# yoxu515/aot-benchmark

Hardware: NVIDIA H100
Metric: frames/sec (480p, 10 obj) (higher is better)
Workload: dtype f32

## Files before the change

### aot_benchmark_b200/csrc/conv_tc.cu

```cuda
#include <type_traits>

#include "common.cuh"
#include "tc_common.cuh"

namespace aotb {
namespace tc {

constexpr int CONV_A_BYTES = 128 * 128;

template <int BN>
__device__ __forceinline__ void wgmma_conv(float* acc, uint64_t a, uint64_t b) {
    if (BN == 256) wgmma_ss_n256(acc, a, b, 1u);
    else if (BN == 128) wgmma_ss_n128(acc, a, b, 1u);
    else wgmma_ss_n64(acc, a, b, 1u);
}

template <int BN>
__device__ __forceinline__ void conv_acc_to_staging(const float* acc, float* stg, int ld) {
    const int warp = threadIdx.x >> 5, lane = threadIdx.x & 31;
    const int row0 = (warp >> 2) * 64 + (warp & 3) * 16 + (lane >> 2), cq = (lane & 3) * 2;
#pragma unroll
    for (int j = 0; j < BN / 2; j += 2)
        *reinterpret_cast<float2*>(stg + (row0 + 8 * ((j >> 1) & 1)) * ld + 8 * (j >> 2) + cq) = make_float2(acc[j], acc[j + 1]);
}

struct ConvTcArgs {
    const float* in;
    const float* bias;
    const float* wscale;
    const float* res;
    float* out;
    int B, H, W, Cin, ldin;
    int Ho, Wo, Cout, ldout, ldres;
    int KH, KW, stride, pad;
    int M, mtiles, nchunks;
    int act;
    int splits;
    int spin;
    int const_w;
    long long* prof;
};

constexpr int AOTB_CONV_CONST_WEIGHTS = 256;
static int g_conv_tiling = 0;
static int g_conv_grid_cap = 0;

struct RowInfo { int pix_base, iy0, ix0, valid; };

template <int BN, int S, int NB>
__device__ __forceinline__ void conv_finish_tile(const ConvTcArgs& a, const uint8_t* smem, int tid, int m0, int n0, int zrank) {
    constexpr int LD = BN + 4, C4 = BN / 4, RSTEP = 256 / C4, ROWS = 128 / S, ITERS = ROWS / RSTEP;
    constexpr int B = NB < ITERS ? NB : ITERS;
    static_assert(ITERS >= 1 && ITERS % B == 0, "finish tiling");
    const int c = (tid % C4) * 4, n = n0 + c;
    const int r0 = zrank * ROWS + tid / C4;
    const float4 b4 = a.bias ? __ldg(reinterpret_cast<const float4*>(a.bias + n)) : make_float4(0.f, 0.f, 0.f, 0.f);
    const float4 s4 = a.wscale ? __ldg(reinterpret_cast<const float4*>(a.wscale + n)) : make_float4(1.f, 1.f, 1.f, 1.f);
    const float* lbase = reinterpret_cast<const float*>(smem) + r0 * LD + c;
    const uint32_t sbase = smem_u32(lbase);
#pragma unroll 1
    for (int i0 = 0; i0 < ITERS; i0 += B) {
        float4 v[B][S], rs[B];
#pragma unroll
        for (int b = 0; b < B; ++b) {
            const int ro = (i0 + b) * RSTEP;
            if (S == 1) {
                v[b][0] = *reinterpret_cast<const float4*>(lbase + ro * LD);
            } else {
#pragma unroll
                for (int z = 0; z < S; ++z) v[b][z] = dsmem_ld_f4(dsmem_addr(sbase + (uint32_t)(ro * LD) * 4u, (uint32_t)z));
            }
            const int m = m0 + r0 + ro;
            rs[b] = (a.res && m < a.M) ? *reinterpret_cast<const float4*>(a.res + (size_t)m * a.ldres + n)
                                       : make_float4(0.f, 0.f, 0.f, 0.f);
        }
#pragma unroll
        for (int b = 0; b < B; ++b) {
            float4 o = v[b][0];
#pragma unroll
            for (int z = 1; z < S; ++z) { o.x += v[b][z].x; o.y += v[b][z].y; o.z += v[b][z].z; o.w += v[b][z].w; }
            o.x = fmaf(o.x, s4.x, b4.x); o.y = fmaf(o.y, s4.y, b4.y); o.z = fmaf(o.z, s4.z, b4.z); o.w = fmaf(o.w, s4.w, b4.w);
            o.x += rs[b].x; o.y += rs[b].y; o.z += rs[b].z; o.w += rs[b].w;
            o.x = apply_act(o.x, a.act); o.y = apply_act(o.y, a.act);
            o.z = apply_act(o.z, a.act); o.w = apply_act(o.w, a.act);
            const int m = m0 + r0 + (i0 + b) * RSTEP;
            if (m < a.M) *reinterpret_cast<float4*>(a.out + (size_t)m * a.ldout + n) = o;
        }
    }
}

__device__ __forceinline__ void prefetch_l1(const void* p) { asm volatile("prefetch.global.L1 [%0];" ::"l"(p)); }

template <int BN, int ACT>
__device__ __forceinline__ void conv_finish_frag(const ConvTcArgs& a, float* acc, const float* bs, int m0, int n0) {
    constexpr bool ROLL = ACT == ACT_GELU || ACT == ACT_SILU;
    constexpr int G = (ROLL || BN == 256) ? 1 : 8, NG = BN / 8, PF = 8;
    const int warp = threadIdx.x >> 5, lane = threadIdx.x & 31;
    const int r = m0 + (warp >> 2) * 64 + (warp & 3) * 16 + (lane >> 2);
    const int c = (lane & 3) * 2;
    const bool ok[2] = {r < a.M, r + 8 < a.M};
    auto res_at = [&](int h, int k) { return a.res + (size_t)(r + 8 * h) * a.ldres + n0 + c + 8 * k; };
    auto prefetch = [&](int k) {
        if (G == 1 && a.res && k < NG) {
            if (ok[0]) prefetch_l1(res_at(0, k));
            if (ok[1]) prefetch_l1(res_at(1, k));
        }
    };
    auto group = [&](int k, int h, float a0, float a1, float2 rs) {
        const int n = c + 8 * k;
        const float2 b2 = *reinterpret_cast<const float2*>(bs + n), s2 = *reinterpret_cast<const float2*>(bs + BN + n);
        float ox = fmaf(a0, s2.x, b2.x), oy = fmaf(a1, s2.y, b2.y);
        ox += rs.x; oy += rs.y;
        ox = apply_act(ox, ACT); oy = apply_act(oy, ACT);
        if (ok[h]) *reinterpret_cast<float2*>(a.out + (size_t)(r + 8 * h) * a.ldout + n0 + n) = make_float2(ox, oy);
    };
#pragma unroll
    for (int k = 0; k < PF; ++k) prefetch(k);
    if constexpr (ROLL) {
#pragma unroll 1
        for (int k = 0; k < NG; ++k) {
            prefetch(k + PF);
            float2 rs[2];
#pragma unroll
            for (int h = 0; h < 2; ++h)
                rs[h] = (a.res && ok[h]) ? *reinterpret_cast<const float2*>(res_at(h, k)) : make_float2(0.f, 0.f);
#pragma unroll
            for (int h = 0; h < 2; ++h) group(k, h, acc[2 * h], acc[2 * h + 1], rs[h]);
#pragma unroll
            for (int i = 0; i < BN / 2 - 4; ++i) acc[i] = acc[i + 4];
        }
    } else {
#pragma unroll
        for (int k0 = 0; k0 < NG; k0 += G) {
            prefetch(k0 + PF);
            float2 rs[G][2];
#pragma unroll
            for (int k = 0; k < G; ++k)
#pragma unroll
                for (int h = 0; h < 2; ++h)
                    rs[k][h] = (a.res && ok[h]) ? *reinterpret_cast<const float2*>(res_at(h, k0 + k)) : make_float2(0.f, 0.f);
#pragma unroll
            for (int k = 0; k < G; ++k)
#pragma unroll
                for (int h = 0; h < 2; ++h) group(k0 + k, h, acc[4 * (k0 + k) + 2 * h], acc[4 * (k0 + k) + 2 * h + 1], rs[k][h]);
        }
    }
}

template <int BN, int STAGES, bool SPLIT, bool PERSIST>
struct ConvSmem {
    static constexpr int A_BYTES = CONV_A_BYTES;
    static constexpr int B_BYTES = BN * 128;
    static constexpr int PARTS = SPLIT ? 2 : 1;
    static constexpr int STAGE_BYTES = PARTS * A_BYTES + PARTS * B_BYTES;
    static constexpr int STG_LD = BN + 4;
    static_assert(128 * STG_LD * 4 <= STAGES * STAGE_BYTES, "staging tile must fit in the operand stages");
    static constexpr int RTABLES = PERSIST ? 2 : 1, BS_FLOATS = PERSIST ? 2 * 2 * BN : 0;
    static constexpr int TOTAL = STAGES * STAGE_BYTES + RTABLES * 128 * (int)sizeof(RowInfo) + BS_FLOATS * 4 + 3 * STAGES * 8 + 1024;
    static_assert(TOTAL <= 227 * 1024, "shared memory of one CTA");
};

template <int BN, int STAGES, bool SPLIT, bool PERSIST>
__global__ void __launch_bounds__(384, 1)
conv_tc_kernel(const __grid_constant__ CUtensorMap tmWh, const __grid_constant__ CUtensorMap tmWl, const ConvTcArgs a) {
    using SM = ConvSmem<BN, STAGES, SPLIT, PERSIST>;
    extern __shared__ uint8_t smem_raw[];
    uint8_t* smem = reinterpret_cast<uint8_t*>((reinterpret_cast<uintptr_t>(smem_raw) + 1023) & ~(uintptr_t)1023);
    RowInfo* rinfo = reinterpret_cast<RowInfo*>(smem + STAGES * SM::STAGE_BYTES);
    float* bsm = reinterpret_cast<float*>(rinfo + SM::RTABLES * 128);
    uint64_t* a_full = reinterpret_cast<uint64_t*>(bsm + SM::BS_FLOATS);
    uint64_t* b_full = a_full + STAGES;
    uint64_t* s_free = b_full + STAGES;

    const int tid = threadIdx.x, warp = tid >> 5;
    const int ntn = a.Cout / BN, ntiles = a.mtiles * ntn;
    const int ntc = !PERSIST ? 1 : (int)blockIdx.x < ntiles ? (ntiles - 1 - (int)blockIdx.x) / (int)gridDim.x + 1 : 0;
    auto tile_m0 = [&](int j) {
        if constexpr (PERSIST) return ((int)(blockIdx.x + j * gridDim.x) / ntn) * 128;
// ... 70 lines not shown
                bs[tid] = a.bias ? __ldg(a.bias + n) : 0.f;
                bs[BN + tid] = a.wscale ? __ldg(a.wscale + n) : 1.f;
            }
#pragma unroll 1
            for (int it = 0; it < nloc; ++it, ++g) {
                const int s = g % STAGES;
                const uint32_t ph = (g / STAGES) & 1;
                mbar_wait_cp(&a_full[s], ph, a.spin);
                mbar_wait_cp(&b_full[s], ph, a.spin);
                if (g == 0 && tid == 0) stamp(3);
                const uint64_t so = (uint64_t)((s * SM::STAGE_BYTES) >> 4);
                const uint64_t ah = dA0 + so, al = ah + (SM::A_BYTES >> 4), bh = dB0 + so, bl = bh + (uint64_t)(SM::B_BYTES >> 4);
                reg_fence<BN / 2>(acc);
                wgmma_fence();
#pragma unroll
                for (int ks = 0; ks < 4; ++ks) {
                    wgmma_conv<BN>(acc, ah + 2 * ks, bh + 2 * ks);
                    if constexpr (SPLIT) {
                        wgmma_conv<BN>(acc, al + 2 * ks, bh + 2 * ks);
                        wgmma_conv<BN>(acc, ah + 2 * ks, bl + 2 * ks);
                    }
                }
                wgmma_commit();
                reg_fence<BN / 2>(acc);
                wgmma_wait<1>();
                if (it > 0) mbar_arrive_warp(&s_free[(g - 1) % STAGES]);
            }
            wgmma_wait<0>();
            reg_fence<BN / 2>(acc);
            if (tid == 0) { if (PERSIST && j == 0) stamp(10); stamp(4); }
            if constexpr (PERSIST) {
                if (nloc > 0) mbar_arrive_warp(&s_free[(g - 1) % STAGES]);
                asm volatile("bar.sync 1, 256;" ::: "memory");
                const int m0 = tile_m0(j), n0 = tile_n0(j);
                switch (a.act) {
                    case ACT_RELU: conv_finish_frag<BN, ACT_RELU>(a, acc, bs, m0, n0); break;
                    case ACT_GELU: conv_finish_frag<BN, ACT_GELU>(a, acc, bs, m0, n0); break;
                    case ACT_SILU: conv_finish_frag<BN, ACT_SILU>(a, acc, bs, m0, n0); break;
                    case ACT_RELU6: conv_finish_frag<BN, ACT_RELU6>(a, acc, bs, m0, n0); break;
                    default: conv_finish_frag<BN, ACT_NONE>(a, acc, bs, m0, n0); break;
                }
                if (tid == 0) { if (j == 0) stamp(8); stamp(9); }
            } else {
                asm volatile("bar.sync 1, 256;" ::: "memory");
                conv_acc_to_staging<BN>(acc, reinterpret_cast<float*>(smem), SM::STG_LD);
                if (tid == 0) stamp(6);
            }
        }
    } else {
        const int p = tid - 256, q = p & 15, rsub = p >> 4;
        const uint32_t soff = rsub * 128 + (((q >> 1) ^ rsub) << 4) + ((q & 1) << 3);
        const float4* in4 = reinterpret_cast<const float4*>(a.in);
        uint32_t off[16];
        int cur_tap = -1, c4 = 0;
        const RowInfo* rows = rinfo;
        auto load_half = [&](int h, auto part_c, float4* v) {
            constexpr int part = decltype(part_c)::value;
            if (part == 0) {
                const int g = h >> 1, j = PERSIST ? g / nloc : 0, it = g - j * nloc;
                if (PERSIST && it == 0) {
                    cur_tap = -1;
                    rows = rinfo + (j & 1) * 128;
                    if (j > 0) {
                        asm volatile("bar.sync 2, 128;" ::: "memory");
                        if (j + 1 < ntc) write_rows(j + 1, p);
                    }
                }
                const int kc = kbeg + it;
                int tap, c0;
                if (cpt > 0) { tap = kc / cpt; c0 = ((kc - tap * cpt) << 6) + q * 4; }
                else { const int k = kc * 64 + q * 4; tap = k / a.Cin; c0 = k - tap * a.Cin; }
                c4 = c0 >> 2;
                if (tap != cur_tap) {
                    cur_tap = tap;
// ... 63 lines not shown
                if (h + 4 < nh) load_half(h + 4, P0{}, v1);
                store_half(h + 2, P0{}, v2);
                if (h + 5 < nh) load_half(h + 5, P1{}, v2);
                store_half(h + 3, P1{}, v0);
            }
            if (h + 4 < nh) {
                if (h + 6 < nh) load_half(h + 6, P0{}, v0);
                store_half(h + 4, P0{}, v1);
                if (h + 7 < nh) load_half(h + 7, P1{}, v1);
                store_half(h + 5, P1{}, v2);
            }
        }
        if (p == 0) stamp(5);
    }
    if constexpr (!PERSIST) {
        __syncwarp();
        cluster_sync_all();
        if (tid == 0) stamp(8);
        if (warp < 8) {
            const int zr = (int)blockIdx.z, m0 = tile_m0(0), n0 = tile_n0(0);
            if (a.splits == 2) conv_finish_tile<BN, 2, 4>(a, smem, tid, m0, n0, zr);
            else if (a.splits == 4) conv_finish_tile<BN, 4, 2>(a, smem, tid, m0, n0, zr);
            else conv_finish_tile<BN, 8, 2>(a, smem, tid, m0, n0, zr);
        }
        if (tid == 0) stamp(9);
        __syncwarp();
        cluster_sync_all();
    } else if (tid == 0 && prof) {
        prof[11] = ntc;
    }
    if (tid == 0) stamp(7);
}

static int make_tmap_weights(CUtensorMap* out, const void* base, int Kpad, int Cout, int BN) {
    PFN_encodeTiled fn = tensor_map_encoder();
    if (!fn) return AOTB_ERR_CUDA;
    cuuint64_t dims[2] = {(cuuint64_t)Kpad, (cuuint64_t)Cout};
    cuuint64_t strides[1] = {(cuuint64_t)Kpad * 2};
    cuuint32_t box[2] = {64, (cuuint32_t)BN};
    cuuint32_t estr[2] = {1, 1};
    CUresult r = fn(out, CU_TENSOR_MAP_DATA_TYPE_FLOAT16, 2, const_cast<void*>(base), dims, strides, box, estr,
                    CU_TENSOR_MAP_INTERLEAVE_NONE, CU_TENSOR_MAP_SWIZZLE_128B, CU_TENSOR_MAP_L2_PROMOTION_L2_256B,
                    CU_TENSOR_MAP_FLOAT_OOB_FILL_NONE);
    if (r != CUDA_SUCCESS) {
        set_error("cuTensorMapEncodeTiled(weights) failed (%d)", (int)r);
        return AOTB_ERR_CUDA;
    }
    return AOTB_OK;
}

static int sm_count() {
    static int n = 0;
    if (n == 0) {
        int dev = 0;
        if (cudaGetDevice(&dev) != cudaSuccess || cudaDeviceGetAttribute(&n, cudaDevAttrMultiProcessorCount, dev) != cudaSuccess)
            n = 132;
    }
    return n;
}

static dim3 conv_grid(const ConvTcArgs& a, int BN) {
    if (a.splits > 1) return dim3(a.mtiles, a.Cout / BN, a.splits);
    const int cap = g_conv_grid_cap > 0 ? g_conv_grid_cap : sm_count();
    return dim3(min(a.mtiles * (a.Cout / BN), cap), 1, 1);
}

template <int BN, int STAGES, bool SPLIT, bool PERSIST>
static int launch_conv_tc_as(const CUtensorMap& th, const CUtensorMap& tl, const ConvTcArgs& a, cudaStream_t st) {
    constexpr int smem = ConvSmem<BN, STAGES, SPLIT, PERSIST>::TOTAL;
    static bool configured = false;
    if (!configured) {
        cudaError_t e = cudaFuncSetAttribute(conv_tc_kernel<BN, STAGES, SPLIT, PERSIST>,
                                             cudaFuncAttributeMaxDynamicSharedMemorySize, smem);
        if (e != cudaSuccess) {
            set_error("aotb_conv2d_nhwc_tc: cudaFuncSetAttribute: %s", cudaGetErrorString(e));
            return AOTB_ERR_CUDA;
        }
        configured = true;
    }
    launch_cluster(conv_tc_kernel<BN, STAGES, SPLIT, PERSIST>, conv_grid(a, BN), dim3(384), smem, st, a.splits, th, tl, a);
    return check_launch("aotb_conv2d_nhwc_tc");
}

template <int BN, int STAGES, bool SPLIT>
static int launch_conv_tc(const CUtensorMap& th, const CUtensorMap& tl, const ConvTcArgs& a, cudaStream_t st) {
    return a.splits > 1 ? launch_conv_tc_as<BN, STAGES, SPLIT, false>(th, tl, a, st)
                        : launch_conv_tc_as<BN, STAGES, SPLIT, true>(th, tl, a, st);
}

}
}

using namespace aotb;

extern "C" int aotb_set_conv_tiling(int mode) {
    AOTB_REQUIRE(mode >= 0 && mode < (1 << 12), "aotb_set_conv_tiling: mode is a 12-bit mask");
    tc::g_conv_tiling = mode;
    return AOTB_OK;
}

extern "C" int aotb_set_conv_grid_cap(int ctas) {
    AOTB_REQUIRE(ctas >= 0, "aotb_set_conv_grid_cap: negative cap");
    tc::g_conv_grid_cap = ctas;
    return AOTB_OK;
}

extern "C" int aotb_conv2d_nhwc_tc(const float* in, const void* wh, const void* wl, const float* bias, const float* wscale,
                                   const float* res, float* out, int B, int H, int W, int Cin, int ldin, int Cout, int ldout, int ldres,
                                   int KH, int KW, int stride, int pad, int act, void* workspace, size_t workspace_bytes,
                                   void* stream) {
    AOTB_REQUIRE(in && wh && out, "aotb_conv2d_nhwc_tc: null pointer");
    const bool split = wl != nullptr;
    const int const_w = (act & tc::AOTB_CONV_CONST_WEIGHTS) ? 1 : 0;
    act &= ~tc::AOTB_CONV_CONST_WEIGHTS;
    AOTB_REQUIRE(Cin % 4 == 0 && Cout % 64 == 0, "aotb_conv2d_nhwc_tc: Cin must be a multiple of 4, Cout of 64");
    AOTB_REQUIRE(act >= aotb::ACT_NONE && act <= aotb::ACT_RELU6, "aotb_conv2d_nhwc_tc: activation %d not supported (0-4)", act);
    AOTB_REQUIRE(ldin % 4 == 0 && ldout % 4 == 0 && (!res || ldres % 4 == 0) && ((uintptr_t)in % 16 == 0) &&
                     ((uintptr_t)out % 16 == 0) && (!res || (uintptr_t)res % 16 == 0) && (!bias || (uintptr_t)bias % 16 == 0) &&
                     (!wscale || (uintptr_t)wscale % 16 == 0),
                 "aotb_conv2d_nhwc_tc: 16-byte alignment required");
    AOTB_REQUIRE((size_t)B * H * W * ldin / 4 < 0xFFFFFFFFull, "aotb_conv2d_nhwc_tc: input larger than 2^32 float4");
    tc::ConvTcArgs a;
    a.in = in; a.bias = bias; a.wscale = wscale; a.res = res; a.out = out;
    a.B = B; a.H = H; a.W = W; a.Cin = Cin; a.ldin = ldin;
    a.Ho = (H + 2 * pad - KH) / stride + 1;
    a.Wo = (W + 2 * pad - KW) / stride + 1;
    AOTB_REQUIRE(a.Ho > 0 && a.Wo > 0, "aotb_conv2d_nhwc_tc: empty output");
    a.Cout = Cout; a.ldout = ldout; a.ldres = ldres; a.KH = KH; a.KW = KW; a.stride = stride; a.pad = pad;
    a.M = B * a.Ho * a.Wo;
    a.mtiles = cdiv(a.M, 128);
    const int K = ((KH * KW * Cin + 63) / 64) * 64;
    a.nchunks = K / 64;
    a.act = act;
    a.const_w = const_w;
    const int mt = cdiv(a.M, 128);
    int BN = 64, best_s = 1;
    const float kGather = 2.5f, kGather1 = 2.0f;
    if ((tc::g_conv_tiling & 1) == 0) {
        float best = 1e30f;
        const int bns[3] = {256, 128, 64};
        const float t_mma[3] = {4.0f, 2.0f, 1.0f}, t_mma1[3] = {4.0f / 3, 2.0f / 3, 1.0f / 3};
        const float t_fin[3] = {8.0f, 4.0f, 2.0f};
        for (int bi = 0; bi < 3; ++bi) {
            const float tf = t_fin[bi] * (bi == 0 && res ? 2.0f : 1.0f);
            if (Cout % bns[bi]) continue;
            const float tm = split ? t_mma[bi] : t_mma1[bi], tc = fmaxf(split ? kGather : kGather1, tm);
            for (int sp = 1; sp <= 8; sp <<= 1) {
                if (sp > a.nchunks) break;
                const int ctas = mt * (Cout / bns[bi]) * sp;
                const int slots = sp == 8 ? 128 : 132;
                if (sp > 1 && ctas > slots) continue;
                float t;
                if (sp == 1) {
                    const int tpc = cdiv(ctas, 132);
                    t = 3.0f + tpc * a.nchunks * tc + tf + (tpc - 1) * fmaxf(0.f, a.nchunks * (tm - tc) + tf);
                } else {
                    t = cdiv(ctas, slots) * (3.0f + cdiv(a.nchunks, sp) * tc + t_fin[bi]);
                }
                if (t < best) { best = t; BN = bns[bi]; best_s = sp; }
            }
        }
    } else {
        if (Cout % 128 == 0 && mt * (Cout / 128) >= 120) BN = 128;
        const int ctas = mt * (Cout / BN);
        if (ctas < 100 && a.nchunks >= 4) {
            best_s = 8;
            while (best_s > 1 && (ctas * best_s > 160 || a.nchunks / best_s < 2)) best_s >>= 1;
        }
    }
    const int force_bn = (tc::g_conv_tiling >> 4) & 15, force_s = (tc::g_conv_tiling >> 8) & 15;
    if (force_bn) {
        BN = 32 << force_bn;
        AOTB_REQUIRE((BN == 64 || BN == 128 || BN == 256) && Cout % BN == 0, "aotb_conv2d_nhwc_tc: forced tile %d invalid", BN);
    }
    a.splits = force_bn ? 1 : best_s;
    if (force_s) {
        AOTB_REQUIRE((force_s == 1 || force_s == 2 || force_s == 4 || force_s == 8) && force_s <= a.nchunks,
                     "aotb_conv2d_nhwc_tc: forced split %d invalid", force_s);
        a.splits = force_s;
    }
    a.spin = (tc::g_conv_tiling & 2) ? 1 : 0;
    a.prof = nullptr;
    if (tc::g_conv_tiling & 4) {
        const dim3 grid = tc::conv_grid(a, BN);
        const size_t need = (size_t)grid.x * grid.y * grid.z * 12 * sizeof(long long);
        AOTB_REQUIRE(workspace && workspace_bytes >= need, "aotb_conv2d_nhwc_tc: profile mode needs %zu workspace bytes", need);
        a.prof = (long long*)workspace;
    }
    CUtensorMap th, tl;
    int rc;
    if ((rc = tc::make_tmap_weights(&th, wh, K, Cout, BN)) != AOTB_OK) return rc;
    cudaStream_t st = (cudaStream_t)stream;
    if (!split) {
        if (BN == 256) return tc::launch_conv_tc<256, 4, false>(th, th, a, st);
        if (BN == 128) return tc::launch_conv_tc<128, 6, false>(th, th, a, st);
        return tc::launch_conv_tc<64, 8, false>(th, th, a, st);
    }
    if ((rc = tc::make_tmap_weights(&tl, wl, K, Cout, BN)) != AOTB_OK) return rc;
    if (BN == 256) return tc::launch_conv_tc<256, 2, true>(th, tl, a, st);
    if (BN == 128) return tc::launch_conv_tc<128, 3, true>(th, tl, a, st);
    return tc::launch_conv_tc<64, 4, true>(th, tl, a, st);
}
```

### aot_benchmark_b200/csrc/tc_common.cuh

```cuda
#pragma once
#include <cuda.h>
#include <cuda_fp16.h>
#include <cuda_runtime.h>
#include <cstdint>

namespace aotb {
namespace tc {

__device__ __forceinline__ uint32_t smem_u32(const void* p) { return (uint32_t)__cvta_generic_to_shared(p); }

__device__ __forceinline__ bool elect_one() {
    uint32_t pred;
    asm volatile(
        "{\n\t.reg .pred P;\n\telect.sync _|P, 0xffffffff;\n\tselp.b32 %0, 1, 0, P;\n\t}\n" : "=r"(pred));
    return pred != 0;
}

__device__ __forceinline__ void mbar_init(uint64_t* bar, uint32_t count) {
    asm volatile("mbarrier.init.shared::cta.b64 [%0], %1;" ::"r"(smem_u32(bar)), "r"(count) : "memory");
}
__device__ __forceinline__ void fence_mbar_init() { asm volatile("fence.mbarrier_init.release.cluster;" ::: "memory"); }
__device__ __forceinline__ void mbar_arrive_warp(uint64_t* bar) {
    __syncwarp();
    if ((threadIdx.x & 31) == 0) asm volatile("mbarrier.arrive.shared::cta.b64 _, [%0];" ::"r"(smem_u32(bar)) : "memory");
// ... 124 lines not shown
        : "+f"(d[0]), "+f"(d[1]), "+f"(d[2]), "+f"(d[3]), "+f"(d[4]), "+f"(d[5]), "+f"(d[6]), "+f"(d[7]),
          "+f"(d[8]), "+f"(d[9]), "+f"(d[10]), "+f"(d[11]), "+f"(d[12]), "+f"(d[13]), "+f"(d[14]), "+f"(d[15]),
          "+f"(d[16]), "+f"(d[17]), "+f"(d[18]), "+f"(d[19]), "+f"(d[20]), "+f"(d[21]), "+f"(d[22]), "+f"(d[23]),
          "+f"(d[24]), "+f"(d[25]), "+f"(d[26]), "+f"(d[27]), "+f"(d[28]), "+f"(d[29]), "+f"(d[30]), "+f"(d[31]),
          "+f"(d[32]), "+f"(d[33]), "+f"(d[34]), "+f"(d[35]), "+f"(d[36]), "+f"(d[37]), "+f"(d[38]), "+f"(d[39]),
          "+f"(d[40]), "+f"(d[41]), "+f"(d[42]), "+f"(d[43]), "+f"(d[44]), "+f"(d[45]), "+f"(d[46]), "+f"(d[47]),
          "+f"(d[48]), "+f"(d[49]), "+f"(d[50]), "+f"(d[51]), "+f"(d[52]), "+f"(d[53]), "+f"(d[54]), "+f"(d[55]),
          "+f"(d[56]), "+f"(d[57]), "+f"(d[58]), "+f"(d[59]), "+f"(d[60]), "+f"(d[61]), "+f"(d[62]), "+f"(d[63]),
          "+f"(d[64]), "+f"(d[65]), "+f"(d[66]), "+f"(d[67]), "+f"(d[68]), "+f"(d[69]), "+f"(d[70]), "+f"(d[71]),
          "+f"(d[72]), "+f"(d[73]), "+f"(d[74]), "+f"(d[75]), "+f"(d[76]), "+f"(d[77]), "+f"(d[78]), "+f"(d[79]),
          "+f"(d[80]), "+f"(d[81]), "+f"(d[82]), "+f"(d[83]), "+f"(d[84]), "+f"(d[85]), "+f"(d[86]), "+f"(d[87]),
          "+f"(d[88]), "+f"(d[89]), "+f"(d[90]), "+f"(d[91]), "+f"(d[92]), "+f"(d[93]), "+f"(d[94]), "+f"(d[95]),
          "+f"(d[96]), "+f"(d[97]), "+f"(d[98]), "+f"(d[99]), "+f"(d[100]), "+f"(d[101]), "+f"(d[102]), "+f"(d[103]),
          "+f"(d[104]), "+f"(d[105]), "+f"(d[106]), "+f"(d[107]), "+f"(d[108]), "+f"(d[109]), "+f"(d[110]), "+f"(d[111]),
          "+f"(d[112]), "+f"(d[113]), "+f"(d[114]), "+f"(d[115]), "+f"(d[116]), "+f"(d[117]), "+f"(d[118]), "+f"(d[119]),
          "+f"(d[120]), "+f"(d[121]), "+f"(d[122]), "+f"(d[123]), "+f"(d[124]), "+f"(d[125]), "+f"(d[126]), "+f"(d[127])
        : "l"(a_desc), "l"(b_desc), "r"(scale_d));
}

__device__ __forceinline__ void wgmma_rs_n64_tb(float* d, const uint32_t* a, uint64_t b_desc) {
    asm volatile(
        "{\n\t.reg .pred p;\n\tsetp.ne.b32 p, 1, 0;\n\t"
        "wgmma.mma_async.sync.aligned.m64n64k16.f32.f16.f16 "
        "{%0, %1, %2, %3, %4, %5, %6, %7, %8, %9, %10, %11, %12, %13, %14, %15, "
        "%16, %17, %18, %19, %20, %21, %22, %23, %24, %25, %26, %27, %28, %29, %30, %31}, "
        "{%32, %33, %34, %35}, %36, p, 1, 1, 1;\n\t}\n"
        : "+f"(d[0]), "+f"(d[1]), "+f"(d[2]), "+f"(d[3]), "+f"(d[4]), "+f"(d[5]), "+f"(d[6]), "+f"(d[7]),
          "+f"(d[8]), "+f"(d[9]), "+f"(d[10]), "+f"(d[11]), "+f"(d[12]), "+f"(d[13]), "+f"(d[14]), "+f"(d[15]),
          "+f"(d[16]), "+f"(d[17]), "+f"(d[18]), "+f"(d[19]), "+f"(d[20]), "+f"(d[21]), "+f"(d[22]), "+f"(d[23]),
          "+f"(d[24]), "+f"(d[25]), "+f"(d[26]), "+f"(d[27]), "+f"(d[28]), "+f"(d[29]), "+f"(d[30]), "+f"(d[31])
        : "r"(a[0]), "r"(a[1]), "r"(a[2]), "r"(a[3]), "l"(b_desc));
}


__device__ __forceinline__ float ex2(float x) {
    float y;
    asm("ex2.approx.ftz.f32 %0, %1;" : "=f"(y) : "f"(x));
    return y;
}
__device__ __forceinline__ uint32_t cvt_h2(float lo, float hi) {
    uint32_t r;
    asm("cvt.rn.f16x2.f32 %0, %1, %2;" : "=r"(r) : "f"(hi), "f"(lo));
    return r;
}

__device__ __forceinline__ void cluster_sync_all() {
    asm volatile("barrier.cluster.arrive.release.aligned;\n\tbarrier.cluster.wait.acquire.aligned;" ::: "memory");
}
__device__ __forceinline__ uint32_t dsmem_addr(uint32_t local_saddr, uint32_t cta_rank) {
    uint32_t r;
    asm volatile("mapa.shared::cluster.u32 %0, %1, %2;" : "=r"(r) : "r"(local_saddr), "r"(cta_rank));
    return r;
}
__device__ __forceinline__ float4 dsmem_ld_f4(uint32_t cluster_saddr) {
    float4 v;
    asm volatile("ld.shared::cluster.v4.f32 {%0, %1, %2, %3}, [%4];"
                 : "=f"(v.x), "=f"(v.y), "=f"(v.z), "=f"(v.w)
                 : "r"(cluster_saddr));
    return v;
}

typedef CUresult (*PFN_encodeTiled)(CUtensorMap*, CUtensorMapDataType, cuuint32_t, void*, const cuuint64_t*,
                                    const cuuint64_t*, const cuuint32_t*, const cuuint32_t*, CUtensorMapInterleave,
                                    CUtensorMapSwizzle, CUtensorMapL2promotion, CUtensorMapFloatOOBfill);
PFN_encodeTiled tensor_map_encoder();

// ... 5 lines not shown
```

### include/aotb200.h

```cpp
#ifndef AOTB200_H
#define AOTB200_H
#include <stddef.h>
#ifdef __cplusplus
extern "C" {
#endif

int aotb_version(void);
const char* aotb_arch(void);
const char* aotb_last_error_string(void);
unsigned long long aotb_launch_count(void);
void aotb_set_pdl(int on);
int aotb_set_conv_tiling(int mode);
int aotb_set_conv_grid_cap(int ctas);

int aotb_conv2d_nhwc_f32(const float* in, const float* w, const float* bias, const float* res, float* out,
                         int B, int H, int W, int Cin, int ldin, int Cout, int ldout, int ldres,
                         int KH, int KW, int stride, int pad, int dil, int act, void* stream);

#define AOTB_CONV_CONST_WEIGHTS 256
int aotb_conv2d_nhwc_tc(const float* in, const void* wh, const void* wl, const float* bias, const float* wscale,
                        const float* res, float* out, int B, int H, int W, int Cin, int ldin, int Cout, int ldout, int ldres,
                        int KH, int KW, int stride, int pad, int act, void* workspace, size_t workspace_bytes,
                        void* stream);

int aotb_linear_f32(const float* in, const float* wt, const float* bias, const float* res, float* out,
                    int M, int K, int ldin, int N, int ldout, int ldres, int act, void* stream);

int aotb_nchw_to_nhwc_f32(const float* in, float* out, int B, int C, int HW, void* stream);
int aotb_nhwc_to_nchw_f32(const float* in, float* out, int B, int C, int HW, void* stream);
int aotb_image_to_nhwc4_f32(const float* in, float* out, int HW, void* stream);
int aotb_image_to_nhwc4_batched_f32(const float* in, float* out, int B, int HW, void* stream);

int aotb_maxpool3x3s2_nhwc_f32(const float* in, float* out, int B, int H, int W, int C, void* stream);

int aotb_dwconv_nhwc_f32(const float* in, const float* w, const float* bias, float* out, int B, int H, int W,
                         int C, int ldin, int ldout, int KH, int KW, int stride, int pad, int dil, int act,
                         void* stream);

int aotb_bilinear_nhwc_f32(const float* in, float* out, int B, int H, int W, int C, int Ho, int Wo,
                           int align_corners, void* stream);

int aotb_eltwise_f32(int op, const float* a, int lda, const float* b, int ldb, float* out, int ldo,
                     int rows, int cols, float scalar, void* stream);

int aotb_layernorm_f32(const float* x, int ldx, const float* gamma, const float* beta, const float* add,
                       int ldadd, float* out, int ldo, float* out2, int ldo2, int rows, int C, void* stream);
// ... 147 lines not shown
```

Baseline: 418.8.

## Add halo-tiled 3x3 conv kernel with register-A wgmma and shared input tile

Adds a specialized kernel for 3x3 stride-1 pad-1 convolutions. Producer warps load an 8x16 spatial output tile plus halo into shared memory once per 64-channel slice, converting to fp16 and optionally a split hi/lo pair. The nine taps are then served from that tile via ldmatrix and register-operand wgmma instead of re-gathering im2col rows per tap. A cost model picks between this path and the existing implicit-GEMM path; it is on by default. The trade-off is a wgmma_wait<0> after every k-group, which serializes MMA issue, plus new tile-shape edge handling.

After: 433.8 (median of 6 runs). 1.04x the previous value.

```diff
diff --git a/aot_benchmark_b200/csrc/conv_tc.cu b/aot_benchmark_b200/csrc/conv_tc.cu
--- a/aot_benchmark_b200/csrc/conv_tc.cu
+++ b/aot_benchmark_b200/csrc/conv_tc.cu
@@ -39,11 +39,13 @@
     int spin;
     int const_w;
     long long* prof;
+    int htx, hti;
 };
 
 constexpr int AOTB_CONV_CONST_WEIGHTS = 256;
 static int g_conv_tiling = 0;
 static int g_conv_grid_cap = 0;
+static int g_conv_halo = 1;
 
 struct RowInfo { int pix_base, iy0, ix0, valid; };
 
@@ -92,13 +94,13 @@
 __device__ __forceinline__ void prefetch_l1(const void* p) { asm volatile("prefetch.global.L1 [%0];" ::"l"(p)); }
 
 template <int BN, int ACT>
-__device__ __forceinline__ void conv_finish_frag(const ConvTcArgs& a, float* acc, const float* bs, int m0, int n0) {
+__device__ __forceinline__ void conv_finish_frag(const ConvTcArgs& a, float* acc, const float* bs, int r, bool ok0, bool ok1,
+                                                 int n0) {
     constexpr bool ROLL = ACT == ACT_GELU || ACT == ACT_SILU;
     constexpr int G = (ROLL || BN == 256) ? 1 : 8, NG = BN / 8, PF = 8;
-    const int warp = threadIdx.x >> 5, lane = threadIdx.x & 31;
-    const int r = m0 + (warp >> 2) * 64 + (warp & 3) * 16 + (lane >> 2);
+    const int lane = threadIdx.x & 31;
     const int c = (lane & 3) * 2;
-    const bool ok[2] = {r < a.M, r + 8 < a.M};
+    const bool ok[2] = {ok0, ok1};
     auto res_at = [&](int h, int k) { return a.res + (size_t)(r + 8 * h) * a.ldres + n0 + c + 8 * k; };
     auto prefetch = [&](int k) {
         if (G == 1 && a.res && k < NG) {
@@ -144,6 +146,18 @@
 #pragma unroll
                 for (int h = 0; h < 2; ++h) group(k0 + k, h, acc[4 * (k0 + k) + 2 * h], acc[4 * (k0 + k) + 2 * h + 1], rs[k][h]);
         }
+    }
+}
+
+template <int BN>
+__device__ __forceinline__ void conv_finish_act(const ConvTcArgs& a, float* acc, const float* bs, int r, bool ok0, bool ok1,
+                                                int n0) {
+    switch (a.act) {
+        case ACT_RELU: conv_finish_frag<BN, ACT_RELU>(a, acc, bs, r, ok0, ok1, n0); break;
+        case ACT_GELU: conv_finish_frag<BN, ACT_GELU>(a, acc, bs, r, ok0, ok1, n0); break;
+        case ACT_SILU: conv_finish_frag<BN, ACT_SILU>(a, acc, bs, r, ok0, ok1, n0); break;
+        case ACT_RELU6: conv_finish_frag<BN, ACT_RELU6>(a, acc, bs, r, ok0, ok1, n0); break;
+        default: conv_finish_frag<BN, ACT_NONE>(a, acc, bs, r, ok0, ok1, n0); break;
     }
 }
 
@@ -280,14 +294,8 @@
             if constexpr (PERSIST) {
                 if (nloc > 0) mbar_arrive_warp(&s_free[(g - 1) % STAGES]);
                 asm volatile("bar.sync 1, 256;" ::: "memory");
-                const int m0 = tile_m0(j), n0 = tile_n0(j);
-                switch (a.act) {
-                    case ACT_RELU: conv_finish_frag<BN, ACT_RELU>(a, acc, bs, m0, n0); break;
-                    case ACT_GELU: conv_finish_frag<BN, ACT_GELU>(a, acc, bs, m0, n0); break;
-                    case ACT_SILU: conv_finish_frag<BN, ACT_SILU>(a, acc, bs, m0, n0); break;
-                    case ACT_RELU6: conv_finish_frag<BN, ACT_RELU6>(a, acc, bs, m0, n0); break;
-                    default: conv_finish_frag<BN, ACT_NONE>(a, acc, bs, m0, n0); break;
-                }
+                const int r = tile_m0(j) + warp * 16 + ((tid & 31) >> 2);
+                conv_finish_act<BN>(a, acc, bs, r, r < a.M, r + 8 < a.M, tile_n0(j));
                 if (tid == 0) { if (j == 0) stamp(8); stamp(9); }
             } else {
                 asm volatile("bar.sync 1, 256;" ::: "memory");
@@ -417,6 +425,205 @@
     if (tid == 0) stamp(7);
 }
 
+constexpr int HALO_PIX = 10 * 18, HALO_PART_BYTES = HALO_PIX * 128;
+
+template <int BN, int STAGES, bool SPLIT>
+struct HaloSmem {
+    static constexpr int PARTS = SPLIT ? 2 : 1;
+    static constexpr int B_BYTES = BN * 128;
+    static constexpr int STAGE_BYTES = PARTS * B_BYTES;
+    static constexpr int HALO_BYTES = PARTS * HALO_PART_BYTES;
+    static constexpr int TOTAL = STAGES * STAGE_BYTES + 2 * HALO_BYTES + 2 * 2 * BN * 4 + (2 * STAGES + 4) * 8 + 1024;
+    static_assert(TOTAL <= 227 * 1024, "shared memory of one CTA");
+};
+
+template <int BN>
+__device__ __forceinline__ void wgmma_rs_conv(float* acc, const uint32_t* a, uint64_t b) {
+    if (BN == 256) wgmma_rs_n256(acc, a, b);
+    else if (BN == 128) wgmma_rs_n128(acc, a, b);
+    else wgmma_rs_n64(acc, a, b);
+}
+
+template <int BN, int STAGES, bool SPLIT>
+__global__ void __launch_bounds__(384, 1)
+conv3x3_halo_kernel(const __grid_constant__ CUtensorMap tmWh, const __grid_constant__ CUtensorMap tmWl, const ConvTcArgs a) {
+    using SM = HaloSmem<BN, STAGES, SPLIT>;
+    constexpr int KG = BN < 256 ? 4 : SPLIT ? 1 : 2;
+    extern __shared__ uint8_t smem_raw[];
+    uint8_t* smem = reinterpret_cast<uint8_t*>((reinterpret_cast<uintptr_t>(smem_raw) + 1023) & ~(uintptr_t)1023);
+    uint8_t* halo = smem + STAGES * SM::STAGE_BYTES;
+    float* bsm = reinterpret_cast<float*>(halo + 2 * SM::HALO_BYTES);
+    uint64_t* b_full = reinterpret_cast<uint64_t*>(bsm + 4 * BN);
+    uint64_t* b_free = b_full + STAGES;
+    uint64_t* h_full = b_free + STAGES;
+    uint64_t* h_free = h_full + 2;
+
+    const int tid = threadIdx.x, warp = tid >> 5, lane = tid & 31;
+    const int ntn = a.Cout / BN, ntiles = a.mtiles * ntn;
+    const int ntc = (int)blockIdx.x < ntiles ? (ntiles - 1 - (int)blockIdx.x) / (int)gridDim.x + 1 : 0;
+    const int ns = a.Cin >> 6, nloc = 9 * ns, nchk = ntc * nloc;
+    auto tile_of = [&](int j, int& b, int& y0, int& x0, int& n0) {
+        const int t = (int)blockIdx.x + j * (int)gridDim.x, mb = t / ntn;
+        n0 = (t - mb * ntn) * BN;
+        b = mb / a.hti;
+        const int r = mb - b * a.hti, ty = r / a.htx;
+        y0 = ty * 8;
+        x0 = (r - ty * a.htx) * 16;
+    };
+    pdl_trigger();
+    if (tid == 0) {
+        for (int s = 0; s < STAGES; ++s) { mbar_init(&b_full[s], 1); mbar_init(&b_free[s], 8); }
+        for (int s = 0; s < 2; ++s) { mbar_init(&h_full[s], 96); mbar_init(&h_free[s], 8); }
+        fence_mbar_init();
+    }
+    __syncthreads();
+    const int npre = a.const_w ? min(STAGES, nchk) : 0;
+    auto issue_b = [&](int g) {
+        const int j = g / nloc, it = g - j * nloc, sl = it / 9, tap = it - sl * 9, s = g % STAGES;
+        int b, y0, x0, n0;
+        tile_of(j, b, y0, x0, n0);
+        uint8_t* Bh = smem + s * SM::STAGE_BYTES;
+        const int k0 = tap * a.Cin + sl * 64;
+        mbar_arrive_expect_tx(&b_full[s], SM::STAGE_BYTES);
+        tma_load_2d(Bh, &tmWh, &b_full[s], k0, n0);
+        if constexpr (SPLIT) tma_load_2d(Bh + SM::B_BYTES, &tmWl, &b_full[s], k0, n0);
+    };
+    if (tid == 256) {
+        tma_prefetch_desc(&tmWh);
+        if constexpr (SPLIT) tma_prefetch_desc(&tmWl);
+        for (int g = 0; g < npre; ++g) issue_b(g);
+    }
+    pdl_wait();
+
+    const int wg = __shfl_sync(0xffffffffu, tid >> 7, 0);
+    if (wg < 2) {
+        const uint64_t dB0 = smem_desc_sw128(smem_u32(smem));
+        const int lx = (lane & 7) + ((lane >> 3) & 1) * 8, lc = lane >> 4;
+        const uint32_t halo_s = smem_u32(halo);
+        int g = 0, u = 0;
+#pragma unroll 1
+        for (int j = 0; j < ntc; ++j) {
+            int b, y0, x0, n0;
+            tile_of(j, b, y0, x0, n0);
+            float acc[BN / 2];
+#pragma unroll
+            for (int i = 0; i < BN / 2; ++i) acc[i] = 0.f;
+            float* bs = bsm + (j & 1) * 2 * BN;
+            if (tid < BN) {
+                bs[tid] = a.bias ? __ldg(a.bias + n0 + tid) : 0.f;
+                bs[BN + tid] = a.wscale ? __ldg(a.wscale + n0 + tid) : 1.f;
+            }
+#pragma unroll 1
+            for (int sl = 0; sl < ns; ++sl, ++u) {
+                const int hb = u & 1;
+                mbar_wait_cp(&h_full[hb], (u >> 1) & 1, a.spin);
+                const uint32_t hbase = halo_s + hb * SM::HALO_BYTES;
+#pragma unroll 1
+                for (int tap = 0; tap < 9; ++tap, ++g) {
+                    const int ky = tap / 3, kx = tap - ky * 3;
+                    const int hp = (warp + ky) * 18 + lx + kx;
+                    const uint32_t rowa = hbase + hp * 128, sw = hp & 7;
+                    const int s = g % STAGES;
+                    mbar_wait_cp(&b_full[s], (g / STAGES) & 1, a.spin);
+                    const uint64_t bh = dB0 + (uint64_t)((s * SM::STAGE_BYTES) >> 4), bl = bh + (uint64_t)(SM::B_BYTES >> 4);
+#pragma unroll
+                    for (int k0 = 0; k0 < 4; k0 += KG) {
+                        uint32_t ah[KG][4], al[KG][4];
+#pragma unroll
+                        for (int k = 0; k < KG; ++k) {
+                            const uint32_t ad = rowa + (((2 * (k0 + k) + lc) ^ sw) << 4);
+                            ldmatrix_x4(ah[k], ad);
+                            if constexpr (SPLIT) ldmatrix_x4(al[k], ad + HALO_PART_BYTES);
+                        }
+                        if (tap == 8 && k0 + KG == 4) mbar_arrive_warp(&h_free[hb]);
+                        reg_fence<BN / 2>(acc);
+                        wgmma_fence();
+#pragma unroll
+                        for (int k = 0; k < KG; ++k) {
+                            const int ks = k0 + k;
+                            wgmma_rs_conv<BN>(acc, ah[k], bh + 2 * ks);
+                            if constexpr (SPLIT) {
+                                wgmma_rs_conv<BN>(acc, al[k], bh + 2 * ks);
+                                wgmma_rs_conv<BN>(acc, ah[k], bl + 2 * ks);
+                            }
+                        }
+                        wgmma_commit();
+                        wgmma_wait<0>();
+                        reg_fence<BN / 2>(acc);
+#pragma unroll
+                        for (int k = 0; k < KG; ++k)
+#pragma unroll
+                            for (int i = 0; i < 4; ++i) {
+                                asm volatile("" : "+r"(ah[k][i])::"memory");
+                                if constexpr (SPLIT) asm volatile("" : "+r"(al[k][i])::"memory");
+                            }
+                    }
+                    mbar_arrive_warp(&b_free[s]);
+                }
+            }
+            asm volatile("bar.sync 1, 256;" ::: "memory");
+            const int oy = y0 + warp, ox = x0 + (lane >> 2);
+            const int r = (b * a.H + oy) * a.W + ox;
+            conv_finish_act<BN>(a, acc, bs, r, oy < a.H && ox < a.W, oy < a.H && ox + 8 < a.W, n0);
+        }
+    } else if (warp == 8) {
+        if (lane == 0) {
+#pragma unroll 1
+            for (int g = npre; g < nchk; ++g) {
+                const int s = g % STAGES;
+                if (g >= STAGES) mbar_wait_cp(&b_free[s], ((g / STAGES) - 1) & 1, a.spin);
+                issue_b(g);
+            }
+        }
+    } else {
+        const int p = tid - 288, q = p & 15, h0 = p >> 4;
+        const float4* in4 = reinterpret_cast<const float4*>(a.in);
+        int u = 0;
+#pragma unroll 1
+        for (int j = 0; j < ntc; ++j) {
+            int b, y0, x0, n0;
+            tile_of(j, b, y0, x0, n0);
+#pragma unroll 1
+            for (int sl = 0; sl < ns; ++sl, ++u) {
+                const int hb = u & 1;
+                if (u >= 2) mbar_wait_cp(&h_free[hb], ((u >> 1) - 1) & 1, a.spin);
+                uint8_t* hh = halo + hb * SM::HALO_BYTES;
+                const int c4 = sl * 16 + q;
+                constexpr int NB = BN == 256 ? 10 : 15;
+#pragma unroll 1
+                for (int i0 = 0; i0 < 30; i0 += NB) {
+                    float4 v[NB];
+#pragma unroll
+                    for (int i = 0; i < NB; ++i) {
+                        const int h = h0 + 6 * (i0 + i), hy = h / 18, hx = h - hy * 18;
+                        const int iy = y0 - 1 + hy, ix = x0 - 1 + hx;
+                        v[i] = (iy >= 0 && iy < a.H && ix >= 0 && ix < a.W)
+                                   ? __ldg(in4 + (((size_t)(b * a.H + iy) * a.W + ix) * a.ldin >> 2) + c4)
+                                   : make_float4(0.f, 0.f, 0.f, 0.f);
+                    }
+#pragma unroll
+                    for (int i = 0; i < NB; ++i) {
+                        const int h = h0 + 6 * (i0 + i);
+                        uint8_t* dst = hh + h * 128 + ((((q >> 1) ^ (h & 7))) << 4) + ((q & 1) << 3);
+                        const __half2 x0h = __floats2half2_rn(v[i].x, v[i].y), x1h = __floats2half2_rn(v[i].z, v[i].w);
+                        uint2 ph;
+                        ph.x = *reinterpret_cast<const uint32_t*>(&x0h); ph.y = *reinterpret_cast<const uint32_t*>(&x1h);
+                        *reinterpret_cast<uint2*>(dst) = ph;
+                        if constexpr (SPLIT) {
+                            const __half2 l0 = __floats2half2_rn(v[i].x - __low2float(x0h), v[i].y - __high2float(x0h));
+                            const __half2 l1 = __floats2half2_rn(v[i].z - __low2float(x1h), v[i].w - __high2float(x1h));
+                            uint2 pl;
+                            pl.x = *reinterpret_cast<const uint32_t*>(&l0); pl.y = *reinterpret_cast<const uint32_t*>(&l1);
+                            *reinterpret_cast<uint2*>(dst + HALO_PART_BYTES) = pl;
+                        }
+                    }
+                }
+                mbar_arrive(&h_full[hb]);
+            }
+        }
+    }
+}
+
 static int make_tmap_weights(CUtensorMap* out, const void* base, int Kpad, int Cout, int BN) {
     PFN_encodeTiled fn = tensor_map_encoder();
     if (!fn) return AOTB_ERR_CUDA;
@@ -473,6 +680,22 @@
                         : launch_conv_tc_as<BN, STAGES, SPLIT, true>(th, tl, a, st);
 }
 
+template <int BN, int STAGES, bool SPLIT>
+static int launch_halo(const CUtensorMap& th, const CUtensorMap& tl, const ConvTcArgs& a, cudaStream_t st) {
+    constexpr int smem = HaloSmem<BN, STAGES, SPLIT>::TOTAL;
+    static bool configured = false;
+    if (!configured) {
+        cudaError_t e = cudaFuncSetAttribute(conv3x3_halo_kernel<BN, STAGES, SPLIT>, cudaFuncAttributeMaxDynamicSharedMemorySize, smem);
+        if (e != cudaSuccess) {
+            set_error("aotb_conv2d_nhwc_tc: cudaFuncSetAttribute: %s", cudaGetErrorString(e));
+            return AOTB_ERR_CUDA;
+        }
+        configured = true;
+    }
+    launch_cluster(conv3x3_halo_kernel<BN, STAGES, SPLIT>, conv_grid(a, BN), dim3(384), smem, st, 1, th, tl, a);
+    return check_launch("aotb_conv2d_nhwc_tc");
+}
+
 }
 }
 
@@ -487,6 +710,12 @@
 extern "C" int aotb_set_conv_grid_cap(int ctas) {
     AOTB_REQUIRE(ctas >= 0, "aotb_set_conv_grid_cap: negative cap");
     tc::g_conv_grid_cap = ctas;
+    return AOTB_OK;
+}
+
+extern "C" int aotb_set_conv_halo(int mode) {
+    AOTB_REQUIRE(mode >= 0 && mode <= 2, "aotb_set_conv_halo: mode is 0, 1 or 2");
+    tc::g_conv_halo = mode;
     return AOTB_OK;
 }
 
@@ -521,8 +750,8 @@
     const int mt = cdiv(a.M, 128);
     int BN = 64, best_s = 1;
     const float kGather = 2.5f, kGather1 = 2.0f;
+    float best = 1e30f;
     if ((tc::g_conv_tiling & 1) == 0) {
-        float best = 1e30f;
         const int bns[3] = {256, 128, 64};
         const float t_mma[3] = {4.0f, 2.0f, 1.0f}, t_mma1[3] = {4.0f / 3, 2.0f / 3, 1.0f / 3};
         const float t_fin[3] = {8.0f, 4.0f, 2.0f};
@@ -566,6 +795,31 @@
     }
     a.spin = (tc::g_conv_tiling & 2) ? 1 : 0;
     a.prof = nullptr;
+    a.htx = a.hti = 0;
+    const bool halo_ok = tc::g_conv_halo && KH == 3 && KW == 3 && stride == 1 && pad == 1 && Cin % 64 == 0 && force_s <= 1 &&
+                         (tc::g_conv_tiling & 4) == 0;
+    int hBN = BN;
+    bool use_halo = false;
+    if (halo_ok) {
+        a.htx = cdiv(W, 16);
+        a.hti = a.htx * cdiv(H, 8);
+        float best_h = 1e30f;
+        const int bns[3] = {256, 128, 64};
+        for (int bi = 0; bi < 3; ++bi) {
+            const int bn = bns[bi];
+            if (Cout % bn || (force_bn && bn != BN)) continue;
+            const float tm = split ? bn / 64 : fmaxf(bn / 192.0f, 1.0f), tf = 2.0f * (bn / 64) * (bn == 256 && res ? 2.0f : 1.0f);
+            const float th = 3.0f + cdiv(B * a.hti * (Cout / bn), 132) * (a.nchunks * tm + tf);
+            if (th < best_h) { best_h = th; hBN = bn; }
+        }
+        use_halo = tc::g_conv_halo == 2 ||
+                   (!force_bn && !force_s && (tc::g_conv_tiling & 1) == 0 && best_h < best);
+    }
+    if (use_halo) {
+        BN = hBN;
+        a.splits = 1;
+        a.mtiles = B * a.hti;
+    }
     if (tc::g_conv_tiling & 4) {
         const dim3 grid = tc::conv_grid(a, BN);
         const size_t need = (size_t)grid.x * grid.y * grid.z * 12 * sizeof(long long);
@@ -576,6 +830,17 @@
     int rc;
     if ((rc = tc::make_tmap_weights(&th, wh, K, Cout, BN)) != AOTB_OK) return rc;
     cudaStream_t st = (cudaStream_t)stream;
+    if (use_halo) {
+        if (!split) {
+            if (BN == 256) return tc::launch_halo<256, 4, false>(th, th, a, st);
+            if (BN == 128) return tc::launch_halo<128, 6, false>(th, th, a, st);
+            return tc::launch_halo<64, 8, false>(th, th, a, st);
+        }
+        if ((rc = tc::make_tmap_weights(&tl, wl, K, Cout, BN)) != AOTB_OK) return rc;
+        if (BN == 256) return tc::launch_halo<256, 2, true>(th, tl, a, st);
+        if (BN == 128) return tc::launch_halo<128, 3, true>(th, tl, a, st);
+        return tc::launch_halo<64, 4, true>(th, tl, a, st);
+    }
     if (!split) {
         if (BN == 256) return tc::launch_conv_tc<256, 4, false>(th, th, a, st);
         if (BN == 128) return tc::launch_conv_tc<128, 6, false>(th, th, a, st);
diff --git a/aot_benchmark_b200/csrc/tc_common.cuh b/aot_benchmark_b200/csrc/tc_common.cuh
--- a/aot_benchmark_b200/csrc/tc_common.cuh
+++ b/aot_benchmark_b200/csrc/tc_common.cuh
@@ -180,6 +180,79 @@
         : "r"(a[0]), "r"(a[1]), "r"(a[2]), "r"(a[3]), "l"(b_desc));
 }
 
+__device__ __forceinline__ void wgmma_rs_n64(float* d, const uint32_t* a, uint64_t b_desc) {
+    asm volatile(
+        "{\n\t.reg .pred p;\n\tsetp.ne.b32 p, 1, 0;\n\t"
+        "wgmma.mma_async.sync.aligned.m64n64k16.f32.f16.f16 "
+        "{%0, %1, %2, %3, %4, %5, %6, %7, %8, %9, %10, %11, %12, %13, %14, %15, "
+        "%16, %17, %18, %19, %20, %21, %22, %23, %24, %25, %26, %27, %28, %29, %30, %31}, "
+        "{%32, %33, %34, %35}, %36, p, 1, 1, 0;\n\t}\n"
+        : "+f"(d[0]), "+f"(d[1]), "+f"(d[2]), "+f"(d[3]), "+f"(d[4]), "+f"(d[5]), "+f"(d[6]), "+f"(d[7]),
+          "+f"(d[8]), "+f"(d[9]), "+f"(d[10]), "+f"(d[11]), "+f"(d[12]), "+f"(d[13]), "+f"(d[14]), "+f"(d[15]),
+          "+f"(d[16]), "+f"(d[17]), "+f"(d[18]), "+f"(d[19]), "+f"(d[20]), "+f"(d[21]), "+f"(d[22]), "+f"(d[23]),
+          "+f"(d[24]), "+f"(d[25]), "+f"(d[26]), "+f"(d[27]), "+f"(d[28]), "+f"(d[29]), "+f"(d[30]), "+f"(d[31])
+        : "r"(a[0]), "r"(a[1]), "r"(a[2]), "r"(a[3]), "l"(b_desc));
+}
+
+__device__ __forceinline__ void wgmma_rs_n128(float* d, const uint32_t* a, uint64_t b_desc) {
+    asm volatile(
+        "{\n\t.reg .pred p;\n\tsetp.ne.b32 p, 1, 0;\n\t"
+        "wgmma.mma_async.sync.aligned.m64n128k16.f32.f16.f16 "
+        "{%0, %1, %2, %3, %4, %5, %6, %7, %8, %9, %10, %11, %12, %13, %14, %15, "
+        "%16, %17, %18, %19, %20, %21, %22, %23, %24, %25, %26, %27, %28, %29, %30, %31, "
+        "%32, %33, %34, %35, %36, %37, %38, %39, %40, %41, %42, %43, %44, %45, %46, %47, "
+        "%48, %49, %50, %51, %52, %53, %54, %55, %56, %57, %58, %59, %60, %61, %62, %63}, "
+        "{%64, %65, %66, %67}, %68, p, 1, 1, 0;\n\t}\n"
+        : "+f"(d[0]), "+f"(d[1]), "+f"(d[2]), "+f"(d[3]), "+f"(d[4]), "+f"(d[5]), "+f"(d[6]), "+f"(d[7]),
+          "+f"(d[8]), "+f"(d[9]), "+f"(d[10]), "+f"(d[11]), "+f"(d[12]), "+f"(d[13]), "+f"(d[14]), "+f"(d[15]),
+          "+f"(d[16]), "+f"(d[17]), "+f"(d[18]), "+f"(d[19]), "+f"(d[20]), "+f"(d[21]), "+f"(d[22]), "+f"(d[23]),
+          "+f"(d[24]), "+f"(d[25]), "+f"(d[26]), "+f"(d[27]), "+f"(d[28]), "+f"(d[29]), "+f"(d[30]), "+f"(d[31]),
+          "+f"(d[32]), "+f"(d[33]), "+f"(d[34]), "+f"(d[35]), "+f"(d[36]), "+f"(d[37]), "+f"(d[38]), "+f"(d[39]),
+          "+f"(d[40]), "+f"(d[41]), "+f"(d[42]), "+f"(d[43]), "+f"(d[44]), "+f"(d[45]), "+f"(d[46]), "+f"(d[47]),
+          "+f"(d[48]), "+f"(d[49]), "+f"(d[50]), "+f"(d[51]), "+f"(d[52]), "+f"(d[53]), "+f"(d[54]), "+f"(d[55]),
+          "+f"(d[56]), "+f"(d[57]), "+f"(d[58]), "+f"(d[59]), "+f"(d[60]), "+f"(d[61]), "+f"(d[62]), "+f"(d[63])
+        : "r"(a[0]), "r"(a[1]), "r"(a[2]), "r"(a[3]), "l"(b_desc));
+}
+
+__device__ __forceinline__ void wgmma_rs_n256(float* d, const uint32_t* a, uint64_t b_desc) {
+    asm volatile(
+        "{\n\t.reg .pred p;\n\tsetp.ne.b32 p, 1, 0;\n\t"
+        "wgmma.mma_async.sync.aligned.m64n256k16.f32.f16.f16 "
+        "{%0, %1, %2, %3, %4, %5, %6, %7, %8, %9, %10, %11, %12, %13, %14, %15, "
+        "%16, %17, %18, %19, %20, %21, %22, %23, %24, %25, %26, %27, %28, %29, %30, %31, "
+        "%32, %33, %34, %35, %36, %37, %38, %39, %40, %41, %42, %43, %44, %45, %46, %47, "
+        "%48, %49, %50, %51, %52, %53, %54, %55, %56, %57, %58, %59, %60, %61, %62, %63, "
+        "%64, %65, %66, %67, %68, %69, %70, %71, %72, %73, %74, %75, %76, %77, %78, %79, "
+        "%80, %81, %82, %83, %84, %85, %86, %87, %88, %89, %90, %91, %92, %93, %94, %95, "
+        "%96, %97, %98, %99, %100, %101, %102, %103, %104, %105, %106, %107, %108, %109, %110, %111, "
+        "%112, %113, %114, %115, %116, %117, %118, %119, %120, %121, %122, %123, %124, %125, %126, %127}, "
+        "{%128, %129, %130, %131}, %132, p, 1, 1, 0;\n\t}\n"
+        : "+f"(d[0]), "+f"(d[1]), "+f"(d[2]), "+f"(d[3]), "+f"(d[4]), "+f"(d[5]), "+f"(d[6]), "+f"(d[7]),
+          "+f"(d[8]), "+f"(d[9]), "+f"(d[10]), "+f"(d[11]), "+f"(d[12]), "+f"(d[13]), "+f"(d[14]), "+f"(d[15]),
+          "+f"(d[16]), "+f"(d[17]), "+f"(d[18]), "+f"(d[19]), "+f"(d[20]), "+f"(d[21]), "+f"(d[22]), "+f"(d[23]),
+          "+f"(d[24]), "+f"(d[25]), "+f"(d[26]), "+f"(d[27]), "+f"(d[28]), "+f"(d[29]), "+f"(d[30]), "+f"(d[31]),
+          "+f"(d[32]), "+f"(d[33]), "+f"(d[34]), "+f"(d[35]), "+f"(d[36]), "+f"(d[37]), "+f"(d[38]), "+f"(d[39]),
+          "+f"(d[40]), "+f"(d[41]), "+f"(d[42]), "+f"(d[43]), "+f"(d[44]), "+f"(d[45]), "+f"(d[46]), "+f"(d[47]),
+          "+f"(d[48]), "+f"(d[49]), "+f"(d[50]), "+f"(d[51]), "+f"(d[52]), "+f"(d[53]), "+f"(d[54]), "+f"(d[55]),
+          "+f"(d[56]), "+f"(d[57]), "+f"(d[58]), "+f"(d[59]), "+f"(d[60]), "+f"(d[61]), "+f"(d[62]), "+f"(d[63]),
+          "+f"(d[64]), "+f"(d[65]), "+f"(d[66]), "+f"(d[67]), "+f"(d[68]), "+f"(d[69]), "+f"(d[70]), "+f"(d[71]),
+          "+f"(d[72]), "+f"(d[73]), "+f"(d[74]), "+f"(d[75]), "+f"(d[76]), "+f"(d[77]), "+f"(d[78]), "+f"(d[79]),
+          "+f"(d[80]), "+f"(d[81]), "+f"(d[82]), "+f"(d[83]), "+f"(d[84]), "+f"(d[85]), "+f"(d[86]), "+f"(d[87]),
+          "+f"(d[88]), "+f"(d[89]), "+f"(d[90]), "+f"(d[91]), "+f"(d[92]), "+f"(d[93]), "+f"(d[94]), "+f"(d[95]),
+          "+f"(d[96]), "+f"(d[97]), "+f"(d[98]), "+f"(d[99]), "+f"(d[100]), "+f"(d[101]), "+f"(d[102]), "+f"(d[103]),
+          "+f"(d[104]), "+f"(d[105]), "+f"(d[106]), "+f"(d[107]), "+f"(d[108]), "+f"(d[109]), "+f"(d[110]), "+f"(d[111]),
+          "+f"(d[112]), "+f"(d[113]), "+f"(d[114]), "+f"(d[115]), "+f"(d[116]), "+f"(d[117]), "+f"(d[118]), "+f"(d[119]),
+          "+f"(d[120]), "+f"(d[121]), "+f"(d[122]), "+f"(d[123]), "+f"(d[124]), "+f"(d[125]), "+f"(d[126]), "+f"(d[127])
+        : "r"(a[0]), "r"(a[1]), "r"(a[2]), "r"(a[3]), "l"(b_desc));
+}
+
+__device__ __forceinline__ void ldmatrix_x4(uint32_t* r, uint32_t saddr) {
+    asm volatile("ldmatrix.sync.aligned.m8n8.x4.shared.b16 {%0, %1, %2, %3}, [%4];"
+                 : "=r"(r[0]), "=r"(r[1]), "=r"(r[2]), "=r"(r[3])
+                 : "r"(saddr)
+                 : "memory");
+}
+
 
 __device__ __forceinline__ float ex2(float x) {
     float y;
diff --git a/include/aotb200.h b/include/aotb200.h
--- a/include/aotb200.h
+++ b/include/aotb200.h
@@ -12,6 +12,7 @@
 void aotb_set_pdl(int on);
 int aotb_set_conv_tiling(int mode);
 int aotb_set_conv_grid_cap(int ctas);
+int aotb_set_conv_halo(int mode);
 
 int aotb_conv2d_nhwc_f32(const float* in, const float* w, const float* bias, const float* res, float* out,
                          int B, int H, int W, int Cin, int ldin, int Cout, int ldout, int ldres,
```
